# yinyunie/Pose2Room

Hardware: AMD Instinct MI355X
Metric: P2RNet train-step samples/sec (T=1024,J=53,bs=32) (higher is better)
Workload: dtype f32; 1 GPU; P2RNet full train step, bs=32/GPU, T=1024, J=53, seeds=512, proposals=128 (BASELINE configs[2]); input=P2RNet_dataloader over SyntheticPoseDataset, global_batch=32, frames=1024, parallelism=dp1

## Files before the change

include/p2r_hip.h:

```cpp
#ifndef P2R_HIP_H
#define P2R_HIP_H

#include <stdint.h>

#ifdef __cplusplus
extern "C" {
#endif

#define P2R_OK 0
#define P2R_EINVAL (-22)

int p2r_abi_version(void);
const char *p2r_build_arch(void);


int p2r_furthest_point_sampling(int b, int n, int m, const float *dataset,
                                float *temp, int *idxs, void *stream);

int p2r_gather_points(int b, int c, int n, int npoints, const float *points,
                      const int *idx, float *out, void *stream);

int p2r_gather_points_grad(int b, int c, int n, int npoints,
                           const float *grad_out, const int *idx,
                           float *grad_points, void *stream);
// ... 63 lines not shown

int p2r_stgcn_gcn_forward(int N, int T, int V, int K, const int *Lk_host,
                          const float *x, const float *W, const uint8_t *nbr,
                          const float *coef, const float *bias_cv, float *z,
                          float *stats_partial, void *stream);

int p2r_stgcn_gcn2_forward(int N, int T, int V, int K, int ltot, const float *x, const float *Wp,
                           const float *coef, const int *stream, int *stream_work,
                           const float *bias_cv, const float *addend, float *z, float *stats_partial,
                           int *n_partials, const float *bwd_u, const unsigned char *bwd_mask,
                           const float *bwd_fin, void *stream_h);

unsigned long long p2r_stgcn_gcn3_signature(int form);
int p2r_stgcn_gcn3_forward(int N, int T, int V, int K, int ltot, int form, const float *x, const float *Wp,
                           const float *coef, const float *bias_cv, const float *addend, float *z,
                           float *stats_partial, int *n_partials, const float *bwd_u,
                           const unsigned char *bwd_mask, const float *bwd_fin, void *stream_h);

int p2r_stgcn_gcn3_data_gradient_masked_addend(int N, int T, int V, int K, int ltot, const float *x,
                                               const float *Wp, const float *coef, const float *addend,
                                               const unsigned char *addend_mask, float *z, float *stats_partial,
                                               const float *bwd_u, const unsigned char *bwd_mask,
                                               const float *bwd_fin, void *stream_h);

int p2r_stgcn_gcn3_coef_grad(int N, int T, int V, int K, int ltot, const float *x, const float *dz,
                             const float *Wp, int n_blocks, float *dcoef_partial, void *stream);

int p2r_stgcn_gcn3_weight_grad(int N, int T, int V, int K, int ltot, const float *x, const float *dz,
                               const float *coef, int n_blocks, float *dw_partial, float *colsum_partial,
                               void *stream);

int p2r_stgcn_gcn_weight_grad(int N, int T, int V, int K, const int *Lk_host,
                              const float *x, const float *dz,
                              const uint8_t *nbr, const float *coef,
                              int n_blocks, float *dw_partial, float *colsum_partial,
                              int colsum_of_x, void *stream);

int p2r_stgcn_gcn_coef_grad(int N, int T, int V, int K, const int *Lk_host,
                            const float *x, const float *dz, const float *Wt,
                            const uint8_t *nbr, const float *coef, int n_blocks,
                            float *dcoef_partial, void *stream);


int p2r_bn_stats(int rows, int L, const float *x, float *partial, void *stream);

int p2r_bn_apply(int N, int C, int L, const float *x, const float *scale,
// ... 218 lines not shown
```

pose2room_amd/_lib.py:

```python
import ctypes
import os
import re

_HERE = os.path.dirname(os.path.abspath(__file__))
LIB_PATH = os.environ.get("P2R_LIB_PATH") or os.path.join(_HERE, "libp2r_hip.so")
HEADER_PATH = os.path.join(os.path.dirname(_HERE), "include", "p2r_hip.h")

ABI_VERSION = 3

_lib = None


class P2RLibraryError(RuntimeError):
    pass


def declared_symbols(header_path=HEADER_PATH):
    with open(header_path) as f:
        text = f.read()
    text = re.sub(r"/\*.*?\*/", "", text, flags=re.S)
    return sorted(set(re.findall(r"\b(p2r_[a-z0-9_]+)\s*\(", text)))


def lib():
    global _lib
    if _lib is None:
        if not os.path.exists(LIB_PATH):
            raise P2RLibraryError(
                f"{LIB_PATH} is missing: build it with `python -c 'import __graft_entry__ as g; g.build()'` "
                "(or `make -C pose2room_amd/csrc`). pose2room_amd has no CPU fallback.")
# ... 47 lines not shown
```

pose2room_amd/csrc/stgcn_gcn3.hip:

```cpp
#include "stgcn_tile.h"

#include "gcn3_sched.inc"

#ifdef P2R_CYCLE_TRACE
__device__ unsigned long long g3_trace[8 * 32];
extern "C" int p2r_debug_g3_trace(unsigned long long *dst) {
  return (int)hipMemcpyFromSymbol(dst, HIP_SYMBOL(g3_trace), sizeof(g3_trace));
}
#define G3_TRACE_TILE(tile) const bool trace_on = blockIdx.x == 7 && (tile) == 7 + 3 * (int)gridDim.x
#define G3_MARK(i) do { if (trace_on && lane == 0) g3_trace[wave * 32 + (i)] = __builtin_readcyclecounter(); } while (0)
#else
#define G3_TRACE_TILE(tile)
#define G3_MARK(i)
#endif
namespace {

constexpr int G3_F = TILE_F, G3_CP = TILE_CP, G3_NPH = TILE_NPH, G3_NW = TILE_NW, G3_SLOTS = TILE_SLOTS;
constexpr int G3_RS = TILE_RS, G3_BUF = TILE_BUF, G3_NV4 = TILE_NV4, G3_PW = TILE_PW;
static_assert(G3_V == TILE_V && G3_K == 11, "schedule generated for another skeleton");

struct G3Params {
  int T;
  int tiles_per_seq, total_tiles;
};

constexpr int g3_slot_joints[2][G3_NW][G3_SLOTS] = {G3_SLOT_JOINTS_0, G3_SLOT_JOINTS_1};
constexpr int g3_plane0[2][G3_NW] = {G3_PLANE0_0, G3_PLANE0_1};
constexpr int g3_first_slot(int form, int w) {
  for (int i = 0; i < G3_SLOTS; ++i)
    if (g3_slot_joints[form][w][i] >= 0) return i;
  return 0;
}
constexpr int g3_wave_joints(int form, int w) {
  int n = 0;
  for (int i = 0; i < G3_SLOTS; ++i) n += g3_slot_joints[form][w][i] >= 0;
  return n;
}
constexpr int G3_ST = 3;

template <int NE, int O0, int O1, int O2, int O3, int O4, int O5>
__device__ __forceinline__ void g3_gather(const char *xl, float (&xv)[6][4]) {
  constexpr int off[6] = {O0, O1, O2, O3, O4, O5};
#pragma unroll
  for (int j = 0; j < NE; ++j)
#pragma unroll
    for (int s = 0; s < 4; ++s) xv[j][s] = *reinterpret_cast<const float *>(xl + off[j] + s * 4 * G3_RS * 4);
}
// ... 48 lines not shown
  {                                                                              \
    float xv_[6][4], cf_[6];                                                     \
    g3_gather<ne, o0, o1, o2, o3, o4, o5>(xl, xv_);                              \
    g3_coefs<ne, c0, c1, c2, c3, c4, c5>(cl, cf_);                               \
    __builtin_amdgcn_sched_barrier(0);                                           \
    G3_MFMA(set, slot)                                                           \
    __builtin_amdgcn_sched_barrier(0);                                           \
    g3_combine<ne>(cf_, xv_, b_cur);                                             \
  }
#define G3_LAST(set, slot)             \
  {                                    \
    __builtin_amdgcn_sched_barrier(0); \
    G3_MFMA(set, slot)                 \
  }
#define G3_END(parity, pieces, plane0)                                                    \
  {                                                                                       \
    if (copy) { _Pragma("unroll") for (int i_ = pieces; i_ < G3_PW; ++i_) dma_piece(i_); } \
    if (parity) {                                                                         \
      _Pragma("unroll") for (int m_ = 0; m_ < 4; ++m_) _Pragma("unroll") for (int s_ = 0; s_ < 4; ++s_) \
          aS[0][m_][s_] = aS[1][m_][s_];                                                  \
    }                                                                                     \
  }

template <int FORM, bool BWD, int WAVE, bool MADD = false>
__device__ __forceinline__ void g3_wave_main(
    const G3Params &p, float *lds, const float *__restrict__ x, const float *__restrict__ Wp,
    const float *__restrict__ addend, float *__restrict__ z, bool want_stats, const float *__restrict__ bwd_u,
    const unsigned char *__restrict__ bwd_mask, const unsigned char *__restrict__ addend_mask = nullptr) {
  constexpr int V = G3_V, RS = G3_RS, BUF = G3_BUF, NW = G3_NW, SLOTS = G3_SLOTS;
  constexpr int wave = WAVE;
  float *rowstat = lds + 2 * BUF;
  float *bias_l = rowstat + NW * 64 * G3_ST;
  float *bstat = bias_l + 64 * V;
  float *coef_l = bstat + 128;

  const int tid = threadIdx.x;
  const int lane = tid & 63;
  const int g = lane >> 4, r = lane & 15;

  constexpr const int (&sj)[SLOTS] = g3_slot_joints[FORM][WAVE];

  const size_t row_stride = (size_t)p.T * V;
  const char *xl0 = reinterpret_cast<const char *>(lds + g * RS + r * V);
  unsigned cl_off = (unsigned)((coef_l - lds) * sizeof(float));
  asm volatile("" : "+v"(cl_off));
  const char *cl = reinterpret_cast<const char *>(lds) + cl_off;

  int doff[G3_PW];
#pragma unroll
  for (int i = 0; i < G3_PW; ++i) {
    const int pc = i * NW + wave;
    const int e = pc * 64 + lane;
    const int row = e / (RS / 4), c4 = e - row * (RS / 4);
    doff[i] = (pc < TILE_PIECES && e < G3_NV4) ? (int)(((size_t)row * row_stride + 4 * c4) * sizeof(float)) : -1;
  }

  f32x4 acc[SLOTS][4];
  float aS[2][4][4];
  float b_cur[4];
  auto load_a = [&](float (&a)[4][4], int k, int ph) { tile_load_a(a, Wp, k, ph, lane); };

  int tile = blockIdx.x;
  if (tile < p.total_tiles) {
    const int seq = tile / p.tiles_per_seq, t0 = (tile % p.tiles_per_seq) * G3_F;
    const float *xr = x + (size_t)seq * 64 * row_stride + (size_t)t0 * V;
#pragma unroll
    for (int i = 0; i < G3_PW; ++i)
      if (doff[i] >= 0) tile_dma16(xr, doff[i], lds + (i * NW + wave) * 256);
  }
  load_a(aS[0], g3_plane0[FORM][WAVE], 0);

  for (; tile < p.total_tiles; tile += gridDim.x) {
    const int seq = tile / p.tiles_per_seq, t0 = (tile % p.tiles_per_seq) * G3_F;
    const float *xg = x + (size_t)seq * 64 * row_stride + (size_t)t0 * V;
    float *zg = z + (size_t)seq * 64 * row_stride + (size_t)t0 * V;
    const float *ag = addend ? addend + (size_t)seq * 64 * row_stride + (size_t)t0 * V : nullptr;
    const float *ug = BWD ? bwd_u + (size_t)seq * 64 * row_stride + (size_t)t0 * V : nullptr;
    const unsigned char *mg = BWD ? bwd_mask + (size_t)seq * 64 * row_stride + (size_t)t0 * V : nullptr;
    const unsigned char *amg = MADD ? addend_mask + (size_t)seq * 64 * row_stride + (size_t)t0 * V : nullptr;
    const int ntile = tile + gridDim.x;
    const bool has_next = ntile < p.total_tiles;
    const int nseq = has_next ? ntile / p.tiles_per_seq : 0, nt0 = has_next ? (ntile % p.tiles_per_seq) * G3_F : 0;
    const float *nxg = x + (size_t)nseq * 64 * row_stride + (size_t)nt0 * V;
    G3_TRACE_TILE(tile);
    G3_MARK(0);

#pragma unroll
    for (int i = 0; i < SLOTS; ++i) {
      const float *bl = bias_l + 4 * g * V + (sj[i] >= 0 ? sj[i] : 0);
#pragma unroll
      for (int m = 0; m < 4; ++m)
#pragma unroll
        for (int q = 0; q < 4; ++q) acc[i][m][q] = bl[(16 * m + q) * V];
    }

#pragma unroll 1
    for (int ph = 0; ph < G3_NPH; ++ph) {
      G3_MARK(1 + 3 * ph);
      asm volatile("s_waitcnt vmcnt(0)" ::: "memory");
      G3_MARK(2 + 3 * ph);
      __syncthreads();
      G3_MARK(3 + 3 * ph);
      float *buf_nxt = lds + ((ph + 1) & 1) * BUF;
      const char *xl = xl0 + (ph & 1) * BUF * sizeof(float);
      const bool copy = ph + 1 < G3_NPH || has_next;
      const float *src = (ph + 1 < G3_NPH) ? xg + (size_t)(ph + 1) * G3_CP * row_stride : nxg;
      auto dma_piece = [&](int i) {
        if (doff[i] >= 0) tile_dma16(src, doff[i], buf_nxt + (i * NW + wave) * 256);
      };

      if constexpr (FORM == 0) {
        if constexpr (WAVE == 0) { G3_BODY_0_0 } else if constexpr (WAVE == 1) { G3_BODY_0_1 }
        else if constexpr (WAVE == 2) { G3_BODY_0_2 } else if constexpr (WAVE == 3) { G3_BODY_0_3 }
        else if constexpr (WAVE == 4) { G3_BODY_0_4 } else if constexpr (WAVE == 5) { G3_BODY_0_5 }
        else if constexpr (WAVE == 6) { G3_BODY_0_6 } else { G3_BODY_0_7 }
      } else {
        if constexpr (WAVE == 0) { G3_BODY_1_0 } else if constexpr (WAVE == 1) { G3_BODY_1_1 }
        else if constexpr (WAVE == 2) { G3_BODY_1_2 } else if constexpr (WAVE == 3) { G3_BODY_1_3 }
        else if constexpr (WAVE == 4) { G3_BODY_1_4 } else if constexpr (WAVE == 5) { G3_BODY_1_5 }
        else if constexpr (WAVE == 6) { G3_BODY_1_6 } else { G3_BODY_1_7 }
      }
    }

    G3_MARK(13);
// ... 119 lines not shown
#pragma unroll
          for (int it = 0; it < (G3_NV4 + NW * 64 - 1) / (NW * 64); ++it) {
            const int e = it * NW * 64 + tid;
            if (e < G3_NV4) {
              const int row = e / (RS / 4), c4 = e - row * (RS / 4);
              float4 v = srow[e];
              if (arow) {
                const float4 ad4 = arow[(size_t)row * (row_stride / 4) + c4];
                v.x += ad4.x; v.y += ad4.y; v.z += ad4.z; v.w += ad4.w;
              }
              zrow[(size_t)row * (row_stride / 4) + c4] = v;
            }
          }
        }
        asm volatile("s_waitcnt lgkmcnt(0)" ::: "memory");
        __builtin_amdgcn_s_barrier();
      }
    }
    G3_MARK(15);
  }

}

template <int FORM, bool BWD, bool MADD = false>
__global__ __launch_bounds__(G3_NW * 64, 2) void gcn3_kernel(
    G3Params p, int ltot, const float *__restrict__ x, const float *__restrict__ Wp, const float *__restrict__ coef,
    const float *__restrict__ bias_cv, const float *__restrict__ addend, float *__restrict__ z,
    float *__restrict__ stats_partial, const float *__restrict__ bwd_u, const unsigned char *__restrict__ bwd_mask,
    const float *__restrict__ bwd_fin, const unsigned char *__restrict__ addend_mask) {
  constexpr int V = G3_V, BUF = G3_BUF, NW = G3_NW;
  extern __shared__ float lds[];
  float *rowstat = lds + 2 * BUF;
  float *bias_l = rowstat + NW * 64 * G3_ST;
  float *bstat = bias_l + 64 * V;
  float *coef_l = bstat + 128;
  const int tid = threadIdx.x;
  for (int e = tid; e < NW * 64 * G3_ST; e += NW * 64) rowstat[e] = 0.f;
  for (int e = tid; e < 64 * V; e += NW * 64) bias_l[e] = bias_cv ? bias_cv[e] : 0.f;
  for (int e = tid; e < ltot * V; e += NW * 64) coef_l[e] = coef[e];
  if (tid < 64) {
    bstat[2 * tid] = BWD ? bwd_fin[tid] : 0.f;
    bstat[2 * tid + 1] = BWD ? bwd_fin[64 + tid] : 1.f;
  }
  __syncthreads();

  const bool want_stats = stats_partial != nullptr;
  switch (__builtin_amdgcn_readfirstlane(tid >> 6)) {
    case 0: g3_wave_main<FORM, BWD, 0, MADD>(p, lds, x, Wp, addend, z, want_stats, bwd_u, bwd_mask, addend_mask); break;
    case 1: g3_wave_main<FORM, BWD, 1, MADD>(p, lds, x, Wp, addend, z, want_stats, bwd_u, bwd_mask, addend_mask); break;
    case 2: g3_wave_main<FORM, BWD, 2, MADD>(p, lds, x, Wp, addend, z, want_stats, bwd_u, bwd_mask, addend_mask); break;
    case 3: g3_wave_main<FORM, BWD, 3, MADD>(p, lds, x, Wp, addend, z, want_stats, bwd_u, bwd_mask, addend_mask); break;
    case 4: g3_wave_main<FORM, BWD, 4, MADD>(p, lds, x, Wp, addend, z, want_stats, bwd_u, bwd_mask, addend_mask); break;
    case 5: g3_wave_main<FORM, BWD, 5, MADD>(p, lds, x, Wp, addend, z, want_stats, bwd_u, bwd_mask, addend_mask); break;
    case 6: g3_wave_main<FORM, BWD, 6, MADD>(p, lds, x, Wp, addend, z, want_stats, bwd_u, bwd_mask, addend_mask); break;
    default: g3_wave_main<FORM, BWD, 7, MADD>(p, lds, x, Wp, addend, z, want_stats, bwd_u, bwd_mask, addend_mask); break;
  }

  if (stats_partial) {
    __syncthreads();
    if constexpr (BWD) {
      tile_write_sums<G3_ST>(rowstat, stats_partial, tid);
    } else if (tid < 64) {
      const int ntiles = (p.total_tiles - (int)blockIdx.x + (int)gridDim.x - 1) / (int)gridDim.x;
      const float per_joint = (float)(ntiles * G3_F);
      float nw[NW], mw[NW], qw[NW];
      float msum = 0.f;
#pragma unroll
      for (int w = 0; w < NW; ++w) {
        const float *e = rowstat + (w * 64 + tid) * G3_ST;
        nw[w] = per_joint * (float)g3_wave_joints(FORM, w);
        const float d = e[0] / nw[w];
        mw[w] = e[2] + d;
        qw[w] = fmaxf(e[1] - e[0] * d, 0.f);
        msum = fmaf(nw[w], mw[w] - mw[0], msum);
      }
      const float n = per_joint * (float)V;
      const float mean = mw[0] + msum / n;
      float m2 = 0.f;
#pragma unroll
      for (int w = 0; w < NW; ++w) m2 += qw[w] + nw[w] * (mw[w] - mean) * (mw[w] - mean);
      float *o = stats_partial + (size_t)blockIdx.x * 192 + 3 * tid;
      o[0] = n; o[1] = mean; o[2] = m2;
    }
  }
}

template <int FORM, bool BWD, bool MADD = false>
int gcn3_launch(const G3Params &p, int ltot, int blocks, size_t lds, const float *x, const float *Wp, const float *coef,
                const float *bias_cv, const float *addend, float *z, float *stats_partial, const float *bwd_u,
                const unsigned char *bwd_mask, const float *bwd_fin, void *stream_h,
                const unsigned char *addend_mask = nullptr) {
  return p2r_launch_big_lds<gcn3_kernel<FORM, BWD, MADD>>(blocks, G3_NW * 64, lds, stream_h, p, ltot, x, Wp, coef, bias_cv,
                                                          addend, z, stats_partial, bwd_u, bwd_mask, bwd_fin, addend_mask);
}

}

extern "C" unsigned long long p2r_stgcn_gcn3_signature(int form) {
  return form == 0 ? G3_SIGNATURE_0 : (form == 1 ? G3_SIGNATURE_1 : 0ull);
}

static int gcn3_forward_impl(int N, int T, int V, int K, int ltot, int form, const float *x, const float *Wp,
                             const float *coef, const float *bias_cv, const float *addend, float *z,
                             float *stats_partial, int *n_partials, const float *bwd_u,
                             const unsigned char *bwd_mask, const float *bwd_fin, const unsigned char *addend_mask,
                             void *stream_h) {
// ... 33 lines not shown
                                       bwd_fin, stream_h);
  return gcn3_launch<1, false>(p, ltot, blocks, lds, x, Wp, coef, bias_cv, addend, z, stats_partial, nullptr, nullptr, nullptr,
                               stream_h);
}

extern "C" int p2r_stgcn_gcn3_forward(int N, int T, int V, int K, int ltot, int form, const float *x, const float *Wp,
                                      const float *coef, const float *bias_cv, const float *addend, float *z,
                                      float *stats_partial, int *n_partials, const float *bwd_u,
                                      const unsigned char *bwd_mask, const float *bwd_fin, void *stream_h) {
  return gcn3_forward_impl(N, T, V, K, ltot, form, x, Wp, coef, bias_cv, addend, z, stats_partial, n_partials, bwd_u, bwd_mask,
                           bwd_fin, nullptr, stream_h);
}

extern "C" int p2r_stgcn_gcn3_data_gradient_masked_addend(int N, int T, int V, int K, int ltot, const float *x,
                                                          const float *Wp, const float *coef, const float *addend,
                                                          const unsigned char *addend_mask, float *z,
                                                          float *stats_partial, const float *bwd_u,
                                                          const unsigned char *bwd_mask, const float *bwd_fin,
                                                          void *stream_h) {
  if (!addend_mask) return P2R_EINVAL;
  return gcn3_forward_impl(N, T, V, K, ltot, 1, x, Wp, coef, nullptr, addend, z, stats_partial, nullptr, bwd_u, bwd_mask,
                           bwd_fin, addend_mask, stream_h);
}
```

pose2room_amd/p2rnet/bn_op.py:

```python
import ctypes

import torch
from torch.autograd import Function

from .. import _lib
from . import handoff, math_mode


def _rows(x):
    N, C = x.shape[0], x.shape[1]
    L = x.numel() // max(N * C, 1)
    return N, C, L


def _stats_partial(x):
    N, C, L = _rows(x)
    part = torch.empty((N, C, 3), dtype=torch.float32, device=x.device)
    with torch.cuda.device(x.device):
        _lib.check(_lib.lib().p2r_bn_stats(N * C, L, _lib.ptr(x), _lib.ptr(part), _lib.current_stream(x.device)),
                   "bn_stats")
    return part


def _stats(x):
# ... 40 lines not shown
    mean = tot[:, 0] / M
    var = (tot[:, 1] / M - mean * mean).clamp_(min=0.0)
    return mean, var, float(M)


def _apply(x, scale, shift, res, relu, want_mask=False):
    N, C, L = _rows(x)
    y = torch.empty_like(x)
    mask = torch.empty(x.shape, dtype=torch.uint8, device=x.device) if (want_mask and relu) else None
    with torch.cuda.device(x.device):
        if relu and want_mask and math_mode.split16() and x.dim() == 4 and N > 0:
            word = math_mode.new_word(x.device)
            _lib.check(_lib.lib().p2r_bn_apply_amax(N, C, L, _lib.ptr(x), _lib.ptr(scale), _lib.ptr(shift), _lib.ptr(res),
                                                    _lib.ptr(y), _lib.ptr(mask), _lib.ptr(word),
                                                    _lib.current_stream(x.device)), "bn_apply_amax")
            math_mode.announce(y, word)
        else:
            _lib.check(_lib.lib().p2r_bn_apply(N, C, L, _lib.ptr(x), _lib.ptr(scale), _lib.ptr(shift), _lib.ptr(res),
                                               int(relu), _lib.ptr(y), _lib.ptr(mask), _lib.current_stream(x.device)),
                       "bn_apply")
    return (y, mask) if want_mask else y


GATE_HOOK = None

OVERLAP_APPLY = True
OVERLAP_REDUCE = True
SIDE_INLINE = False
_SIDE = {}


def _side_stream(dev):
    key = (dev.type, dev.index if dev.index is not None else torch.cuda.current_device())
    st = _SIDE.get(key)
    if st is None:
        st = _SIDE[key] = torch.cuda.Stream(device=dev, priority=-1)
    return st


class BNLink(object):
    __slots__ = ('u', 'mask', 'fin', 'versions', 'used')

    def __init__(self):
        self.u = self.mask = self.fin = self.versions = None
        self.used = 0

    def attach(self, u, mask, fin):
        self.u, self.mask, self.fin = u, mask, fin
        self.versions = (u._version, mask._version, fin._version)

    def intact(self):
        return (self.u is not None and self.versions is not None and
                self.versions == (self.u._version, self.mask._version, self.fin._version))


class _FusedBNAct(Function):

    @staticmethod
    def forward(ctx, x, weight, bias, res, fin, relu, link=None, lazy_res=False):
        x = x.contiguous()
        res_c = res.contiguous() if res is not None else None
        y, mask = _apply(x, fin[2], fin[3], res_c, relu, want_mask=True)
        ctx.save_for_backward(x, mask, fin)
        ctx.relu = relu
        ctx.split = math_mode.split16() and relu and x.dim() == 4
        ctx.has_res = res is not None
        ctx.lazy_res = bool(lazy_res) and relu and res is not None
        ctx.link = link if relu else None
        if ctx.link is not None:
            link.attach(x, mask, fin)
        return y

    @staticmethod
    def backward(ctx, dy):
        x, mask, fin = ctx.saved_tensors
        mean, invstd, kscale = fin[0], fin[1], fin[2]
        mode = 3 if ctx.relu else 0
        dy = dy.contiguous()
        N, C, L = _rows(x)
        dev = x.device
        lib = _lib.lib()
        link, part, ready = ctx.link, None, None
        sums = handoff.take(dy, 'bn_sums') if link is not None else None
        if sums is not None and sums[0] is link:
            _, part, ready = sums
# ... 29 lines not shown
                                                    _lib.ptr(invstd), _lib.ptr(kscale), _lib.ptr(tot_[2]), _lib.ptr(tot_[3]),
                                                    mode, None, None, _lib.ptr(dx_), _lib.ptr(dres_),
                                                    _lib.current_stream(dev)), "bn_bwd_apply")
            return tot_, dx_, dres_, word_

        if side_ok and SIDE_INLINE:
            tot, dx, dres, word = apply_pass()
        elif side_ok:
            main, side = torch.cuda.current_stream(dev), _side_stream(dev)
            side.wait_event(ready)
            with torch.cuda.stream(side):
                tot, dx, dres, word = apply_pass()
                done = torch.cuda.Event()
                done.record(side)
            main.wait_event(done)
            for t_ in (tot, dx, dres, word):
                if t_ is not None:
                    t_.record_stream(main)
        else:
            tot, dx, dres, word = apply_pass()
        if ctx.lazy_res:
            handoff.put(dy, 'res_mask', mask)
            dres = dy
        return dx, tot[1], tot[0], dres, None, None, None, None


class _EvalBNAct(Function):

    @staticmethod
    def forward(ctx, x, scale, shift, res, relu):
        x = x.contiguous()
        y = _apply(x, scale.contiguous(), shift.contiguous(), res.contiguous() if res is not None else None, relu)
        ctx.save_for_backward(x, y, scale)
        ctx.relu, ctx.has_res = relu, res is not None
        return y

    @staticmethod
    def backward(ctx, dy):
        x, y, scale = ctx.saved_tensors
        g = dy * (y > 0) if ctx.relu else dy
        dims = [d for d in range(dy.dim()) if d != 1]
        dscale = dshift = None
        if ctx.needs_input_grad[1]:
            dscale = (g.double() * x).sum(dims).float()
        if ctx.needs_input_grad[2]:
            dshift = g.double().sum(dims).float()
        dx = g * scale.view(1, -1, *([1] * (dy.dim() - 2))) if ctx.needs_input_grad[0] else None
        return dx, dscale, dshift, (g if ctx.has_res else None), None


def supported(x, bn):
    return x.is_cuda and x.dtype == torch.float32 and bn.affine and bn.track_running_stats and x.dim() >= 3


def fused_bn_act(x, bn, res=None, relu=True, stats=None, link=None, lazy_res=False):
    if bn.training:
        part = _stats_partial(x.contiguous()) if stats is None else stats
        fin = finalize(part, x.numel() // x.shape[1], bn)
        if GATE_HOOK is not None and relu:
            GATE_HOOK(bn, x, fin[2], fin[3], res)
        y = _FusedBNAct.apply(x, bn.weight, bn.bias, res, fin, relu, link, lazy_res)
        if link is not None and relu:
            y._p2r_bn_link = link
        return y
    invstd = torch.rsqrt(bn.running_var + bn.eps)
    scale = bn.weight * invstd
    shift = bn.bias - bn.running_mean * scale
    if GATE_HOOK is not None and relu:
        GATE_HOOK(bn, x, scale.detach(), shift.detach(), res)
    return _EvalBNAct.apply(x, scale, shift, res, relu)
```

pose2room_amd/p2rnet/gcn_op.py:

```python
import ctypes

import torch
from torch.autograd import Function

from .. import _lib
from . import bn_op, gcn_tables, handoff, math_mode

_N_BLOCKS = 256


class GraphTables:

    def __init__(self, A):
        self.K, self.V = int(A.shape[0]), int(A.shape[1])
        self.nbr_c, self.gidx_c, self.Lk_c = gcn_tables.build(A, transpose=False)
        self.nbr_r, self.gidx_r, self.Lk_r = gcn_tables.build(A, transpose=True)
        self.LkA_c = (ctypes.c_int * self.K)(*self.Lk_c)
        self.LkA_r = (ctypes.c_int * self.K)(*self.Lk_r)
        self.stream_c = self.stream_r = None
        if self.V == 53 and self.K < 15:
            try:
                sc = gcn_tables.build_stream(self.nbr_c, self.gidx_c, self.Lk_c)[0]
                sr = gcn_tables.build_stream(self.nbr_r, self.gidx_r, self.Lk_r)[0]
                self.stream_c, self.stream_r = torch.from_numpy(sc), torch.from_numpy(sr)
# ... 67 lines not shown
        _lib.check(_lib.lib().p2r_stgcn_gcn_forward(
            N, T, V, tables.K, LkA, _lib.ptr(x), _lib.ptr(W), _lib.ptr(nbr), _lib.ptr(coef),
            _lib.ptr(bias_cv), _lib.ptr(z), _lib.ptr(part), _lib.current_stream(x.device)), "stgcn_gcn_forward")
    return (z, part) if want_stats else z


def permute_planes(W3):
    K = W3.shape[0]
    return W3.reshape(K, 4, 16, 4, 4, 4).permute(0, 3, 1, 5, 2, 4).contiguous()


USE_GEN3 = True
SPLIT_WEIGHT_GRAD = True
SPLIT_COEF_GRAD = True


def _gen3_able(x, z, addend, tables, bwd=None):
    return (USE_GEN3 and tables.gen3 and x.shape[0] > 0 and x.shape[2] % 16 == 0 and x.data_ptr() % 16 == 0
            and z.data_ptr() % 16 == 0 and (addend is None or addend.data_ptr() % 16 == 0)
            and (bwd is None or (bwd[0].data_ptr() % 16 == 0 and bwd[1].data_ptr() % 4 == 0)))


def _gcn2_forward(x, Wp, coef, stream, bias_cv, tables, want_stats=False, addend=None, bwd=None, form=None,
                  addend_mask=None):
    N, C, T, V = x.shape
    z = torch.empty_like(x)
    lib = _lib.lib()
    part = None
    ltot = coef.shape[0]
    with torch.cuda.device(x.device):
        st = _lib.current_stream(x.device)
        gen3 = form is not None and _gen3_able(x, z, addend, tables, bwd)
        if addend_mask is not None and not (gen3 and form == 1 and addend_mask.data_ptr() % 4 == 0):
            addend = addend * (addend_mask != 0)
            addend_mask = None
        if want_stats:
            part = torch.empty((min(N * ((T + 15) // 16), 256), C, 3 if gen3 and bwd is None else 2),
                               dtype=torch.float32, device=x.device)
        if gen3 and addend_mask is not None:
            bu, bm, bf = (bwd[0], bwd[1], bwd[2].contiguous()) if bwd is not None else (None, None, None)
            _lib.check(lib.p2r_stgcn_gcn3_data_gradient_masked_addend(
                N, T, V, tables.K, ltot, _lib.ptr(x), _lib.ptr(Wp), _lib.ptr(coef), _lib.ptr(addend), _lib.ptr(addend_mask),
                _lib.ptr(z), _lib.ptr(part), _lib.ptr(bu), _lib.ptr(bm), _lib.ptr(bf), st),
                "stgcn_gcn3_data_gradient_masked_addend")
            return (z, part) if want_stats else z
        if gen3:
            bu, bm, bf = (bwd[0], bwd[1], bwd[2].contiguous()) if bwd is not None else (None, None, None)
            _lib.check(lib.p2r_stgcn_gcn3_forward(N, T, V, tables.K, ltot, int(form), _lib.ptr(x), _lib.ptr(Wp),
                                                  _lib.ptr(coef), _lib.ptr(bias_cv), _lib.ptr(addend), _lib.ptr(z),
                                                  _lib.ptr(part), None, _lib.ptr(bu), _lib.ptr(bm), _lib.ptr(bf), st),
                       "stgcn_gcn3_forward")
            return (z, part) if want_stats else z
        work = torch.empty_like(stream)
        bu, bm, bf = (bwd[0], bwd[1], bwd[2].contiguous()) if bwd is not None else (None, None, None)
        _lib.check(lib.p2r_stgcn_gcn2_forward(N, T, V, tables.K, ltot, _lib.ptr(x), _lib.ptr(Wp), _lib.ptr(coef),
                                              _lib.ptr(stream), _lib.ptr(work), _lib.ptr(bias_cv), _lib.ptr(addend),
                                              _lib.ptr(z), _lib.ptr(part), None, _lib.ptr(bu), _lib.ptr(bm),
                                              _lib.ptr(bf), st), "stgcn_gcn2_forward")
    return (z, part) if want_stats else z


# ... 76 lines not shown
    return (z, part) if want_stats else z


def _gcn3h_data_gradient(dz, sp, coef, tables, addend, addend_mask, dz_word):
    N, C, T, V = dz.shape
    dx = torch.empty_like(dz)
    with torch.cuda.device(dz.device):
        _lib.check(_lib.lib().p2r_stgcn_gcn3h_data_gradient(
            N, T, V, tables.K, coef.shape[0], _lib.ptr(dz), _lib.ptr(sp.wh), _lib.ptr(sp.winv), _lib.ptr(coef),
            _lib.ptr(addend), _lib.ptr(addend_mask), _lib.ptr(dx), _lib.ptr(dz_word), _lib.current_stream(dz.device)),
            "stgcn_gcn3h_data_gradient")
    return dx


class _GraphConv(Function):
    @staticmethod
    def forward(ctx, x, weight, coef_c, coef_r, bias_cv, tables, want_stats=False, with_residual=False,
                bn_link=None, wp_f=None, wp_b=None, lazy_res=False, split=None):
        dev = x.device
        t = tables.on(dev)
        x = x.contiguous()
        W = weight.contiguous()
        ctx.split = ctx.x_word = None
        if split is None and math_mode.split16() and _gen3h_able(x, tables):
            W3 = W.view(tables.K, 64, 64)
            split = (SplitPlanes(*split_planes(W3, tables.pairs_c)),
                     SplitPlanes(*split_planes(W3, tables.pairs_r, transposed=True)),
                     SplitPlanes(*split_planes_coef_grad(W3)))
        if split is not None and _gen3h_able(x, tables):
            ctx.split = split
            ctx.x_word = math_mode.range_word(x)
            out = _gcn3h_forward(x, split[0], coef_c.contiguous(), bias_cv.contiguous(), tables, want_stats, ctx.x_word)
        elif tables.gen2:
            out = _gcn2_forward(x, wp_f if wp_f is not None else permute_planes(W.view(tables.K, 64, 64)),
                                coef_c.contiguous(), t['stream_c'], bias_cv.contiguous(), tables, want_stats, form=0)
        else:
            out = _gcn_forward(x, W, t['nbr_c'], coef_c.contiguous(), tables.LkA_c, bias_cv.contiguous(), tables,
                               want_stats)
        ctx.save_for_backward(x, W, coef_c, coef_r)
        ctx.tables = tables
        ctx.bn_link = bn_link
        ctx.wp_b = wp_b
        ctx.wp_f = wp_f
        ctx.n_out = 2 if want_stats else 1
        ctx.lazy_res = bool(lazy_res) and with_residual
        if want_stats:
            ctx.mark_non_differentiable(out[1])
        if with_residual:
            out = (out if want_stats else (out,)) + (x.view_as(x),)
        return out

    @staticmethod
    def backward(ctx, dz, *rest):
        x, W, coef_c, coef_r = ctx.saved_tensors
        dres = rest[ctx.n_out - 1] if len(rest) >= ctx.n_out else None
        dres_mask = None
        if ctx.lazy_res and dres is not None:
            dres = dres.contiguous()
# ... 194 lines not shown
```

pose2room_amd/p2rnet/modules/stgcn.py:

```python
import torch
import torch.nn as nn

from ..registers import MODULES
from .stgcn_layers import Graph, st_gcn_block
from .sub_modules import SingleConv


def _point_mlp(cin, width, cout):
    return nn.Sequential(SingleConv(cin, width, kernel_size=1, order='cbr', padding=0, ndim=1),
                         SingleConv(width, width, kernel_size=1, order='cbr', padding=0, ndim=1),
                         SingleConv(width, cout, kernel_size=1, order='c', padding=0, ndim=1))


@MODULES.register_module
class STGCN(nn.Module):
    def __init__(self, cfg, optim_spec=None):
        super().__init__()
        self.optim_spec = optim_spec

        self.graph = Graph(layout='virtualroom', strategy='spatial', max_hop=5)
        self.register_buffer('A', torch.tensor(self.graph.A, dtype=torch.float32, requires_grad=False))

        self.n_seeds = cfg.config['data']['num_seeds']
        self.origin_joint_id = cfg.dataset_config.origin_joint_id
# ... 85 lines not shown
            torch.arange(-self.knn // 2, self.knn // 2, device=device).unsqueeze(0)
        win = win.clamp_(0, n_frames - 1)
        offs = hip[:, win] - hip.unsqueeze(2)
        pe = self._mlp(self.pos_embed, offs.reshape(n_batch, n_frames * self.knn, 3).transpose(1, 2).contiguous(), self.knn)
        from .. import seed_op
        pe = pe.view(n_batch, -1, n_frames, self.knn)
        fused = seed_op.short_rows_supported(pe)
        pe = seed_op.mean_last(pe) if fused else pe.mean(dim=3)
        rel = input_joints - input_joints[:, :, self.origin_joint_id:self.origin_joint_id + 1]
        sk = self._mlp(self.sk_feat, rel.reshape(n_batch, n_frames * n_joints, 3).transpose(1, 2).contiguous(), n_joints,
                       add_ct=pe)
        return sk.view(n_batch, -1, n_frames, n_joints)

    def forward(self, input_joints, end_points=None):
        end_points = {} if end_points is None else end_points
        n_batch, n_frames, n_joints, n_dim = input_joints.size()
        seed_inds = self._select_seeds(input_joints[:, :, self.origin_joint_id])

        x = self.embed(input_joints)
        blocks = self.st_gcn_networks
        tables = blocks[0].gcn.tables
        if tables is not None and tables.gen2 and all(b.chainable(x, self.A) for b in blocks):
            from ..gcn_op import prepare_chain
            for gcn, prep in zip(blocks, prepare_chain(blocks, self.A, self.edge_importance, tables, frames=x.shape[2])):
                x, _ = gcn(x, prep.Aeff, prepared=prep)
        else:
            for gcn, importance in zip(blocks, self.edge_importance):
                x, _ = gcn(x, self.A * importance)

        seed_skeleton = torch.gather(
            input_joints, 1, seed_inds[:, :, None, None].expand(n_batch, self.n_seeds, n_joints, n_dim))
        if self.n_seeds < n_frames:
            from .. import seed_op
            if seed_op.seed_rows_supported(x, seed_inds):
                rows = seed_op.seed_rows(x, seed_inds)
            else:
                rows = x.permute(0, 2, 1, 3)[torch.arange(n_batch, device=x.device)[:, None], seed_inds]
            seed_features = torch.nn.functional.linear(
                rows.reshape(n_batch, self.n_seeds, -1),
                self.conv_joint.weight.squeeze(-1), self.conv_joint.bias)
        else:
            x = x.transpose(2, 3).reshape(n_batch, -1, n_frames)
            seed_features = self.conv_joint(x).transpose(1, 2)
            seed_features = torch.gather(
                seed_features, 1, seed_inds.unsqueeze(-1).expand(n_batch, self.n_seeds, seed_features.size(-1)))
        end_points['seed_inds'] = seed_inds
        end_points['seed_skeleton'] = seed_skeleton[..., :3]
        end_points['seed_features'] = seed_features
# ... 2 lines not shown
```

pose2room_amd/p2rnet/modules/stgcn_layers.py:

```python
from collections import deque

import numpy as np
import torch
import torch.nn as nn

_VIRTUALROOM_BONES = [
    (0, 1), (1, 3), (3, 5), (5, 19), (0, 2), (2, 4), (4, 6), (6, 20), (0, 7), (7, 8), (8, 9),
    (9, 10), (10, 21), (10, 22), (8, 11), (11, 13), (13, 15), (15, 17), (8, 12), (12, 14),
    (14, 16), (16, 18), (17, 23), (23, 24), (24, 25), (17, 26), (26, 27), (27, 28), (17, 29),
    (29, 30), (30, 31), (17, 32), (32, 33), (33, 34), (17, 35), (35, 36), (36, 37), (18, 38),
    (38, 39), (39, 40), (18, 41), (41, 42), (42, 43), (18, 44), (44, 45), (45, 46), (18, 47),
    (47, 48), (48, 49), (18, 50), (50, 51), (51, 52)]

_LAYOUTS = {'virtualroom': dict(num_node=53, bones=_VIRTUALROOM_BONES, center=0)}


def hop_distance(num_node, edges, max_hop):
    nbr = [[] for _ in range(num_node)]
    for i, j in edges:
        if i != j:
            nbr[i].append(j)
            nbr[j].append(i)
    hop = np.full((num_node, num_node), np.inf)
    for s in range(num_node):
# ... 108 lines not shown
        if not residual:
            self.residual = _zero
        elif in_channels == out_channels and stride == 1:
            self.residual = _iden
        else:
            self.residual = nn.Sequential(
                nn.Conv2d(in_channels, out_channels, kernel_size=1, stride=(stride, 1)),
                nn.BatchNorm2d(out_channels))
        self.relu = nn.ReLU(inplace=True)

    fused_bn = True
    fused_tconv = True
    lazy_residual_grad = True
    chain_input = False

    def chainable(self, x, A):
        if not (self.fused_bn and x.is_cuda and self.tcn[4].p == 0):
            return False
        from .. import bn_op, gcn_op, tconv_op
        return (self.training and self.fused_tconv and self.gcn.tables is not None and self.gcn.fused
                and gcn_op.supported(x, self.gcn.conv.weight, A) and bn_op.supported(x, self.tcn[0])
                and tconv_op.supported(x, self.tcn[0], self.tcn[2]))

    def forward(self, x, A, prepared=None):
        res = self.residual(x)
        if self.fused_bn and x.is_cuda and self.tcn[4].p == 0:
            from .. import bn_op, gcn_op, tconv_op
            chain = self.chainable(x, A)
            assert chain or prepared is None
            lazy = False
            if chain:
                if self.residual is _iden and x.requires_grad:
                    in_link = getattr(x, '_p2r_bn_link', None) if self.chain_input else None
                    lazy = self.lazy_residual_grad and self.tcn[3].training
                    (z, zstats, res), A = self.gcn(x, A, want_stats=True, with_residual=True, bn_link=in_link,
                                                   prepared=prepared, lazy_res=lazy)
                else:
                    (z, zstats), A = self.gcn(x, A, want_stats=True, prepared=prepared)
                wp = (prepared.tcn_wp_f, prepared.tcn_wp_b) if prepared is not None and z.shape[3] == 53 else None
                u, ustats = tconv_op.bn_relu_tconv(z, self.tcn[0], self.tcn[2], stats=zstats, want_stats=True, wp=wp)
                res_t = res if torch.is_tensor(res) else None
                return bn_op.fused_bn_act(u, self.tcn[3], res_t, relu=True, stats=ustats, link=bn_op.BNLink(),
                                          lazy_res=lazy), A
            x, A = self.gcn(x, A)
            if bn_op.supported(x, self.tcn[0]):
                if self.fused_tconv and tconv_op.supported(x, self.tcn[0], self.tcn[2]):
                    u = tconv_op.bn_relu_tconv(x, self.tcn[0], self.tcn[2])
                else:
                    h = bn_op.fused_bn_act(x, self.tcn[0], None, relu=True)
                    u = self.tcn[2](h)
                res_t = res if torch.is_tensor(res) else None
                return bn_op.fused_bn_act(u, self.tcn[3], res_t, relu=True), A
        else:
            x, A = self.gcn(x, A)
        x = self.tcn(x) + res
        return self.relu(x), A
```

Baseline: 799.4 samples/s.

## Defer block-output BN apply and fuse it into next gcn3 forward load

Instead of running a standalone BatchNorm scale/shift + residual + ReLU pass at the end of each chained st_gcn block, the apply is recorded as a deferred handoff and executed inside the next block's gen3 graph-conv forward kernel. Each tile is transformed in LDS after loading, and the kernel also writes the materialized activation and the ReLU mask. This removes one kernel launch and one full read/write pass of the activation per intermediate block. In exchange it adds residual loads and extra stores inside the GEMM pipeline, which may lengthen the per-phase critical path. Consumers that cannot fuse fall back to a standalone apply.

```diff
diff --git a/include/p2r_hip.h b/include/p2r_hip.h
--- a/include/p2r_hip.h
+++ b/include/p2r_hip.h
@@ -109,6 +109,11 @@
                                                const unsigned char *addend_mask, float *z, float *stats_partial,
                                                const float *bwd_u, const unsigned char *bwd_mask,
                                                const float *bwd_fin, void *stream_h);
+
+int p2r_stgcn_gcn3_forward_xform(int N, int T, int V, int K, int ltot, const float *t, const float *scale,
+                                 const float *shift, const float *res, float *x_next, unsigned char *mask,
+                                 const float *Wp, const float *coef, const float *bias_cv, float *z,
+                                 float *stats_partial, int *n_partials, void *stream_h);
 
 int p2r_stgcn_gcn3_coef_grad(int N, int T, int V, int K, int ltot, const float *x, const float *dz,
                              const float *Wp, int n_blocks, float *dcoef_partial, void *stream);
diff --git a/pose2room_amd/_lib.py b/pose2room_amd/_lib.py
--- a/pose2room_amd/_lib.py
+++ b/pose2room_amd/_lib.py
@@ -6,6 +6,7 @@
 LIB_PATH = os.environ.get("P2R_LIB_PATH") or os.path.join(_HERE, "libp2r_hip.so")
 HEADER_PATH = os.path.join(os.path.dirname(_HERE), "include", "p2r_hip.h")
 
+P2R_EINVAL = -22
 ABI_VERSION = 3
 
 _lib = None
diff --git a/pose2room_amd/csrc/stgcn_gcn3.hip b/pose2room_amd/csrc/stgcn_gcn3.hip
--- a/pose2room_amd/csrc/stgcn_gcn3.hip
+++ b/pose2room_amd/csrc/stgcn_gcn3.hip
@@ -13,6 +13,9 @@
 #define G3_TRACE_TILE(tile)
 #define G3_MARK(i)
 #endif
+#ifndef G3X_RES_WARM
+#define G3X_RES_WARM 0
+#endif
 namespace {
 
 constexpr int G3_F = TILE_F, G3_CP = TILE_CP, G3_NPH = TILE_NPH, G3_NW = TILE_NW, G3_SLOTS = TILE_SLOTS;
@@ -23,6 +26,13 @@
   int T;
   int tiles_per_seq, total_tiles;
 };
+struct G3Xform {
+  const float *scale, *shift;
+  const float *res;
+  float *y;
+  unsigned char *mask;
+};
+typedef float g3_f4v __attribute__((ext_vector_type(4)));
 
 constexpr int g3_slot_joints[2][G3_NW][G3_SLOTS] = {G3_SLOT_JOINTS_0, G3_SLOT_JOINTS_1};
 constexpr int g3_plane0[2][G3_NW] = {G3_PLANE0_0, G3_PLANE0_1};
@@ -117,11 +127,11 @@
     }                                                                                     \
   }
 
-template <int FORM, bool BWD, int WAVE, bool MADD = false>
+template <int FORM, bool BWD, int WAVE, bool MADD = false, int XF = 0>
 __device__ __forceinline__ void g3_wave_main(
     const G3Params &p, float *lds, const float *__restrict__ x, const float *__restrict__ Wp,
     const float *__restrict__ addend, float *__restrict__ z, bool want_stats, const float *__restrict__ bwd_u,
-    const unsigned char *__restrict__ bwd_mask, const unsigned char *__restrict__ addend_mask = nullptr) {
+    const unsigned char *__restrict__ bwd_mask, const unsigned char *__restrict__ addend_mask, const G3Xform &xf) {
   constexpr int V = G3_V, RS = G3_RS, BUF = G3_BUF, NW = G3_NW, SLOTS = G3_SLOTS;
   constexpr int wave = WAVE;
   float *rowstat = lds + 2 * BUF;
@@ -155,6 +165,7 @@
   float b_cur[4];
   auto load_a = [&](float (&a)[4][4], int k, int ph) { tile_load_a(a, Wp, k, ph, lane); };
 
+  float xwarm = 0.f;
   int tile = blockIdx.x;
   if (tile < p.total_tiles) {
     const int seq = tile / p.tiles_per_seq, t0 = (tile % p.tiles_per_seq) * G3_F;
@@ -177,6 +188,8 @@
     const bool has_next = ntile < p.total_tiles;
     const int nseq = has_next ? ntile / p.tiles_per_seq : 0, nt0 = has_next ? (ntile % p.tiles_per_seq) * G3_F : 0;
     const float *nxg = x + (size_t)nseq * 64 * row_stride + (size_t)nt0 * V;
+    const size_t xf_tile = (size_t)seq * 64 * row_stride + (size_t)t0 * V;
+    const size_t xf_ntile = (size_t)nseq * 64 * row_stride + (size_t)nt0 * V;
     G3_TRACE_TILE(tile);
     G3_MARK(0);
 
@@ -192,9 +205,52 @@
 #pragma unroll 1
     for (int ph = 0; ph < G3_NPH; ++ph) {
       G3_MARK(1 + 3 * ph);
+      constexpr int XR4 = RS / 4, XIT = (XR4 + 31) / 32;
+      const int xcol = lane & 31, xrow = 2 * wave + (lane >> 5);
+      const size_t xf_off = xf_tile + (size_t)(G3_CP * ph + xrow) * row_stride + 4 * xcol;
+      g3_f4v xres[XF == 2 ? XIT : 1];
+      if constexpr (XF == 2) {
+        const g3_f4v *r4 = reinterpret_cast<const g3_f4v *>(xf.res + xf_off);
+#pragma unroll
+        for (int it = 0; it < XIT; ++it)
+          if (32 * it + 31 < XR4 || 32 * it + xcol < XR4) xres[it] = __builtin_nontemporal_load(r4 + 32 * it);
+      }
       asm volatile("s_waitcnt vmcnt(0)" ::: "memory");
+      if constexpr (XF == 2 && G3X_RES_WARM) asm volatile("" : "+v"(xwarm));
       G3_MARK(2 + 3 * ph);
       __syncthreads();
+      if constexpr (XF != 0) {
+        const int ch = G3_CP * ph + xrow;
+        const float sc = bstat[2 * ch], sh = bstat[2 * ch + 1];
+        float4 *rp = reinterpret_cast<float4 *>(lds + (ph & 1) * BUF + xrow * RS) + xcol;
+        g3_f4v *y4 = reinterpret_cast<g3_f4v *>(xf.y + xf_off);
+        uchar4 *m4 = reinterpret_cast<uchar4 *>(xf.mask + xf_off);
+#pragma unroll
+        for (int it = 0; it < XIT; ++it)
+          if (32 * it + 31 < XR4 || 32 * it + xcol < XR4) {
+            float4 v = rp[32 * it];
+            v.x = fmaf(v.x, sc, sh); v.y = fmaf(v.y, sc, sh); v.z = fmaf(v.z, sc, sh); v.w = fmaf(v.w, sc, sh);
+            if constexpr (XF == 2) {
+              v.x += xres[it].x; v.y += xres[it].y; v.z += xres[it].z; v.w += xres[it].w;
+            }
+            v.x = fmaxf(v.x, 0.f); v.y = fmaxf(v.y, 0.f); v.z = fmaxf(v.z, 0.f); v.w = fmaxf(v.w, 0.f);
+            rp[32 * it] = v;
+            __builtin_nontemporal_store(g3_f4v{v.x, v.y, v.z, v.w}, y4 + 32 * it);
+            m4[32 * it] = make_uchar4(v.x > 0.f, v.y > 0.f, v.z > 0.f, v.w > 0.f);
+          }
+        asm volatile("s_waitcnt lgkmcnt(0)" ::: "memory");
+        __builtin_amdgcn_s_barrier();
+        if constexpr (XF == 2 && G3X_RES_WARM) {
+          if (ph + 1 < G3_NPH || has_next) {
+            const float *wp = xf.res + (ph + 1 < G3_NPH ? xf_off + (size_t)G3_CP * row_stride
+                                                        : xf_ntile + (size_t)xrow * row_stride + 4 * xcol);
+#pragma unroll
+            for (int it = 0; it < XIT; ++it)
+              if (32 * it + 31 < XR4 || 32 * it + xcol < XR4)
+                asm volatile("global_load_dword %0, %1, off offset:%2" : "+v"(xwarm) : "v"(wp), "n"(512 * it) : "memory");
+          }
+        }
+      }
       G3_MARK(3 + 3 * ph);
       float *buf_nxt = lds + ((ph + 1) & 1) * BUF;
       const char *xl = xl0 + (ph & 1) * BUF * sizeof(float);
@@ -360,6 +416,31 @@
 
 }
 
+template <int FORM>
+__device__ __forceinline__ void g3_merge_moments(const G3Params &p, const float *rowstat, float *stats_partial, int tid) {
+  constexpr int V = G3_V, NW = G3_NW;
+  const int ntiles = (p.total_tiles - (int)blockIdx.x + (int)gridDim.x - 1) / (int)gridDim.x;
+  const float per_joint = (float)(ntiles * G3_F);
+  float nw[NW], mw[NW], qw[NW];
+  float msum = 0.f;
+#pragma unroll
+  for (int w = 0; w < NW; ++w) {
+    const float *e = rowstat + (w * 64 + tid) * G3_ST;
+    nw[w] = per_joint * (float)g3_wave_joints(FORM, w);
+    const float d = e[0] / nw[w];
+    mw[w] = e[2] + d;
+    qw[w] = fmaxf(e[1] - e[0] * d, 0.f);
+    msum = fmaf(nw[w], mw[w] - mw[0], msum);
+  }
+  const float n = per_joint * (float)V;
+  const float mean = mw[0] + msum / n;
+  float m2 = 0.f;
+#pragma unroll
+  for (int w = 0; w < NW; ++w) m2 += qw[w] + nw[w] * (mw[w] - mean) * (mw[w] - mean);
+  float *o = stats_partial + (size_t)blockIdx.x * 192 + 3 * tid;
+  o[0] = n; o[1] = mean; o[2] = m2;
+}
+
 template <int FORM, bool BWD, bool MADD = false>
 __global__ __launch_bounds__(G3_NW * 64, 2) void gcn3_kernel(
     G3Params p, int ltot, const float *__restrict__ x, const float *__restrict__ Wp, const float *__restrict__ coef,
@@ -383,15 +464,16 @@
   __syncthreads();
 
   const bool want_stats = stats_partial != nullptr;
+  const G3Xform no_xf{};
   switch (__builtin_amdgcn_readfirstlane(tid >> 6)) {
-    case 0: g3_wave_main<FORM, BWD, 0, MADD>(p, lds, x, Wp, addend, z, want_stats, bwd_u, bwd_mask, addend_mask); break;
-    case 1: g3_wave_main<FORM, BWD, 1, MADD>(p, lds, x, Wp, addend, z, want_stats, bwd_u, bwd_mask, addend_mask); break;
-    case 2: g3_wave_main<FORM, BWD, 2, MADD>(p, lds, x, Wp, addend, z, want_stats, bwd_u, bwd_mask, addend_mask); break;
-    case 3: g3_wave_main<FORM, BWD, 3, MADD>(p, lds, x, Wp, addend, z, want_stats, bwd_u, bwd_mask, addend_mask); break;
-    case 4: g3_wave_main<FORM, BWD, 4, MADD>(p, lds, x, Wp, addend, z, want_stats, bwd_u, bwd_mask, addend_mask); break;
-    case 5: g3_wave_main<FORM, BWD, 5, MADD>(p, lds, x, Wp, addend, z, want_stats, bwd_u, bwd_mask, addend_mask); break;
-    case 6: g3_wave_main<FORM, BWD, 6, MADD>(p, lds, x, Wp, addend, z, want_stats, bwd_u, bwd_mask, addend_mask); break;
-    default: g3_wave_main<FORM, BWD, 7, MADD>(p, lds, x, Wp, addend, z, want_stats, bwd_u, bwd_mask, addend_mask); break;
+    case 0: g3_wave_main<FORM, BWD, 0, MADD>(p, lds, x, Wp, addend, z, want_stats, bwd_u, bwd_mask, addend_mask, no_xf); break;
+    case 1: g3_wave_main<FORM, BWD, 1, MADD>(p, lds, x, Wp, addend, z, want_stats, bwd_u, bwd_mask, addend_mask, no_xf); break;
+    case 2: g3_wave_main<FORM, BWD, 2, MADD>(p, lds, x, Wp, addend, z, want_stats, bwd_u, bwd_mask, addend_mask, no_xf); break;
+    case 3: g3_wave_main<FORM, BWD, 3, MADD>(p, lds, x, Wp, addend, z, want_stats, bwd_u, bwd_mask, addend_mask, no_xf); break;
+    case 4: g3_wave_main<FORM, BWD, 4, MADD>(p, lds, x, Wp, addend, z, want_stats, bwd_u, bwd_mask, addend_mask, no_xf); break;
+    case 5: g3_wave_main<FORM, BWD, 5, MADD>(p, lds, x, Wp, addend, z, want_stats, bwd_u, bwd_mask, addend_mask, no_xf); break;
+    case 6: g3_wave_main<FORM, BWD, 6, MADD>(p, lds, x, Wp, addend, z, want_stats, bwd_u, bwd_mask, addend_mask, no_xf); break;
+    default: g3_wave_main<FORM, BWD, 7, MADD>(p, lds, x, Wp, addend, z, want_stats, bwd_u, bwd_mask, addend_mask, no_xf); break;
   }
 
   if (stats_partial) {
@@ -420,6 +502,45 @@
       float *o = stats_partial + (size_t)blockIdx.x * 192 + 3 * tid;
       o[0] = n; o[1] = mean; o[2] = m2;
     }
+  }
+}
+
+template <bool RES>
+__global__ __launch_bounds__(G3_NW * 64, 2) void gcn3x_kernel(
+    G3Params p, int ltot, const float *__restrict__ t, G3Xform xf, const float *__restrict__ Wp,
+    const float *__restrict__ coef, const float *__restrict__ bias_cv, float *__restrict__ z,
+    float *__restrict__ stats_partial) {
+  constexpr int V = G3_V, BUF = G3_BUF, NW = G3_NW, XF = RES ? 2 : 1;
+  extern __shared__ float lds[];
+  float *rowstat = lds + 2 * BUF;
+  float *bias_l = rowstat + NW * 64 * G3_ST;
+  float *bstat = bias_l + 64 * V;
+  float *coef_l = bstat + 128;
+  const int tid = threadIdx.x;
+  for (int e = tid; e < NW * 64 * G3_ST; e += NW * 64) rowstat[e] = 0.f;
+  for (int e = tid; e < 64 * V; e += NW * 64) bias_l[e] = bias_cv ? bias_cv[e] : 0.f;
+  for (int e = tid; e < ltot * V; e += NW * 64) coef_l[e] = coef[e];
+  if (tid < 64) {
+    bstat[2 * tid] = xf.scale[tid];
+    bstat[2 * tid + 1] = xf.shift[tid];
+  }
+  __syncthreads();
+
+  const bool want_stats = stats_partial != nullptr;
+  switch (__builtin_amdgcn_readfirstlane(tid >> 6)) {
+    case 0: g3_wave_main<0, false, 0, false, XF>(p, lds, t, Wp, nullptr, z, want_stats, nullptr, nullptr, nullptr, xf); break;
+    case 1: g3_wave_main<0, false, 1, false, XF>(p, lds, t, Wp, nullptr, z, want_stats, nullptr, nullptr, nullptr, xf); break;
+    case 2: g3_wave_main<0, false, 2, false, XF>(p, lds, t, Wp, nullptr, z, want_stats, nullptr, nullptr, nullptr, xf); break;
+    case 3: g3_wave_main<0, false, 3, false, XF>(p, lds, t, Wp, nullptr, z, want_stats, nullptr, nullptr, nullptr, xf); break;
+    case 4: g3_wave_main<0, false, 4, false, XF>(p, lds, t, Wp, nullptr, z, want_stats, nullptr, nullptr, nullptr, xf); break;
+    case 5: g3_wave_main<0, false, 5, false, XF>(p, lds, t, Wp, nullptr, z, want_stats, nullptr, nullptr, nullptr, xf); break;
+    case 6: g3_wave_main<0, false, 6, false, XF>(p, lds, t, Wp, nullptr, z, want_stats, nullptr, nullptr, nullptr, xf); break;
+    default: g3_wave_main<0, false, 7, false, XF>(p, lds, t, Wp, nullptr, z, want_stats, nullptr, nullptr, nullptr, xf); break;
+  }
+
+  if (stats_partial) {
+    __syncthreads();
+    if (tid < 64) g3_merge_moments<0>(p, rowstat, stats_partial, tid);
   }
 }
 
@@ -499,3 +620,35 @@
   return gcn3_forward_impl(N, T, V, K, ltot, 1, x, Wp, coef, nullptr, addend, z, stats_partial, nullptr, bwd_u, bwd_mask,
                            bwd_fin, addend_mask, stream_h);
 }
+
+extern "C" int p2r_stgcn_gcn3_forward_xform(int N, int T, int V, int K, int ltot, const float *t, const float *scale,
+                                            const float *shift, const float *res, float *x_next, unsigned char *mask,
+                                            const float *Wp, const float *coef, const float *bias_cv, float *z,
+                                            float *stats_partial, int *n_partials, void *stream_h) {
+  if (N < 0 || T <= 0 || V != G3_V || K != G3_K || ltot <= 0) return P2R_EINVAL;
+  if (T % G3_F != 0 || T > (1 << 20)) return P2R_EINVAL;
+  if (((uintptr_t)t % 16) != 0 || ((uintptr_t)z % 16) != 0 || ((uintptr_t)res % 16) != 0 ||
+      ((uintptr_t)x_next % 16) != 0 || ((uintptr_t)mask % 4) != 0)
+    return P2R_EINVAL;
+  if (n_partials) *n_partials = 0;
+  if (N == 0) return P2R_OK;
+  G3Params p;
+  p.T = T;
+  p.tiles_per_seq = T / G3_F;
+  const long long tiles = (long long)N * p.tiles_per_seq;
+  if (tiles > 0x7fffffffLL) return P2R_EINVAL;
+  p.total_tiles = (int)tiles;
+  const int blocks = (int)(tiles < 256 ? tiles : 256);
+  if (n_partials) *n_partials = blocks;
+  if (!z) return P2R_OK;
+  if (!t || !scale || !shift || !x_next || !mask || !Wp || !coef) return P2R_EINVAL;
+  const size_t lds = (size_t)2 * G3_BUF * sizeof(float) + (size_t)G3_NW * 64 * G3_ST * sizeof(float) +
+                     (size_t)64 * V * sizeof(float) + 128 * sizeof(float) + (size_t)ltot * V * sizeof(float);
+  if (lds > 160 * 1024) return P2R_EINVAL;
+  const G3Xform xf = {scale, shift, res, x_next, mask};
+  if (res)
+    return p2r_launch_big_lds<gcn3x_kernel<true>>(blocks, G3_NW * 64, lds, stream_h, p, ltot, t, xf, Wp, coef, bias_cv, z,
+                                                  stats_partial);
+  return p2r_launch_big_lds<gcn3x_kernel<false>>(blocks, G3_NW * 64, lds, stream_h, p, ltot, t, xf, Wp, coef, bias_cv, z,
+                                                 stats_partial);
+}
diff --git a/pose2room_amd/p2rnet/bn_op.py b/pose2room_amd/p2rnet/bn_op.py
--- a/pose2room_amd/p2rnet/bn_op.py
+++ b/pose2room_amd/p2rnet/bn_op.py
@@ -86,6 +86,49 @@
     return (y, mask) if want_mask else y
 
 
+DEFER_APPLY = True
+DEFER_COUNTS = {'fused': 0, 'standalone': 0}
+_warned_standalone = False
+
+
+def note_standalone(why):
+    global _warned_standalone
+    DEFER_COUNTS['standalone'] += 1
+    if not _warned_standalone:
+        _warned_standalone = True
+        import warnings
+        warnings.warn("bn_op: a deferred BatchNorm apply pass ran as a standalone launch (" + why + "); the step is "
+                      "correct but loses the fusion", RuntimeWarning, stacklevel=3)
+
+
+class DeferredApply(object):
+    __slots__ = ('t', 'scale', 'shift', 'res', 'mask')
+
+    def __init__(self, t, scale, shift, res, mask):
+        self.t, self.scale, self.shift, self.res, self.mask = t, scale, shift, res, mask
+
+    def run(self, y):
+        N, C, L = _rows(self.t)
+        with torch.cuda.device(y.device):
+            _lib.check(_lib.lib().p2r_bn_apply(N, C, L, _lib.ptr(self.t), _lib.ptr(self.scale), _lib.ptr(self.shift),
+                                               _lib.ptr(self.res), 1, _lib.ptr(y), _lib.ptr(self.mask),
+                                               _lib.current_stream(y.device)), "bn_apply")
+
+
+def materialize(y):
+    d = handoff.take(y, 'bn_deferred') if torch.is_tensor(y) else None
+    if d is not None:
+        note_standalone("its consumer is not a chainable st_gcn block")
+        d.run(y)
+    return y
+
+
+def defer_ok(x, tables):
+    from . import gcn_op
+    return (DEFER_APPLY and gcn_op.USE_GEN3 and tables is not None and tables.gen3 and not math_mode.split16()
+            and x.dim() == 4 and x.shape[0] > 0 and x.shape[2] % 16 == 0)
+
+
 GATE_HOOK = None
 
 OVERLAP_APPLY = True
@@ -121,10 +164,15 @@
 class _FusedBNAct(Function):
 
     @staticmethod
-    def forward(ctx, x, weight, bias, res, fin, relu, link=None, lazy_res=False):
+    def forward(ctx, x, weight, bias, res, fin, relu, link=None, lazy_res=False, defer=False):
         x = x.contiguous()
         res_c = res.contiguous() if res is not None else None
-        y, mask = _apply(x, fin[2], fin[3], res_c, relu, want_mask=True)
+        if defer and relu and x.dim() == 4 and x.shape[0] > 0 and not math_mode.split16():
+            y = torch.empty_like(x)
+            mask = torch.empty(x.shape, dtype=torch.uint8, device=x.device)
+            handoff.put(y, 'bn_deferred', DeferredApply(x, fin[2], fin[3], res_c, mask))
+        else:
+            y, mask = _apply(x, fin[2], fin[3], res_c, relu, want_mask=True)
         ctx.save_for_backward(x, mask, fin)
         ctx.relu = relu
         ctx.split = math_mode.split16() and relu and x.dim() == 4
@@ -200,7 +248,7 @@
         if ctx.lazy_res:
             handoff.put(dy, 'res_mask', mask)
             dres = dy
-        return dx, tot[1], tot[0], dres, None, None, None, None
+        return dx, tot[1], tot[0], dres, None, None, None, None, None
 
 
 class _EvalBNAct(Function):
@@ -231,13 +279,13 @@
     return x.is_cuda and x.dtype == torch.float32 and bn.affine and bn.track_running_stats and x.dim() >= 3
 
 
-def fused_bn_act(x, bn, res=None, relu=True, stats=None, link=None, lazy_res=False):
+def fused_bn_act(x, bn, res=None, relu=True, stats=None, link=None, lazy_res=False, defer=False):
     if bn.training:
         part = _stats_partial(x.contiguous()) if stats is None else stats
         fin = finalize(part, x.numel() // x.shape[1], bn)
         if GATE_HOOK is not None and relu:
             GATE_HOOK(bn, x, fin[2], fin[3], res)
-        y = _FusedBNAct.apply(x, bn.weight, bn.bias, res, fin, relu, link, lazy_res)
+        y = _FusedBNAct.apply(x, bn.weight, bn.bias, res, fin, relu, link, lazy_res, defer)
         if link is not None and relu:
             y._p2r_bn_link = link
         return y
diff --git a/pose2room_amd/p2rnet/gcn_op.py b/pose2room_amd/p2rnet/gcn_op.py
--- a/pose2room_amd/p2rnet/gcn_op.py
+++ b/pose2room_amd/p2rnet/gcn_op.py
@@ -113,7 +113,7 @@
 
 
 def _gcn2_forward(x, Wp, coef, stream, bias_cv, tables, want_stats=False, addend=None, bwd=None, form=None,
-                  addend_mask=None):
+                  addend_mask=None, deferred=None):
     N, C, T, V = x.shape
     z = torch.empty_like(x)
     lib = _lib.lib()
@@ -128,6 +128,20 @@
         if want_stats:
             part = torch.empty((min(N * ((T + 15) // 16), 256), C, 3 if gen3 and bwd is None else 2),
                                dtype=torch.float32, device=x.device)
+        if deferred is not None:
+            if gen3 and form == 0 and bwd is None and addend is None:
+                d = deferred
+                rc = lib.p2r_stgcn_gcn3_forward_xform(N, T, V, tables.K, ltot, _lib.ptr(d.t), _lib.ptr(d.scale),
+                                                      _lib.ptr(d.shift), _lib.ptr(d.res), _lib.ptr(x), _lib.ptr(d.mask),
+                                                      _lib.ptr(Wp), _lib.ptr(coef), _lib.ptr(bias_cv), _lib.ptr(z),
+                                                      _lib.ptr(part), None, st)
+                if rc == 0:
+                    bn_op.DEFER_COUNTS['fused'] += 1
+                    return (z, part) if want_stats else z
+                if rc != _lib.P2R_EINVAL:
+                    _lib.check(rc, "stgcn_gcn3_forward_xform")
+            bn_op.note_standalone("the graph conv that consumes it does not run on the fused third-generation forward")
+            deferred.run(x)
         if gen3 and addend_mask is not None:
             bu, bm, bf = (bwd[0], bwd[1], bwd[2].contiguous()) if bwd is not None else (None, None, None)
             _lib.check(lib.p2r_stgcn_gcn3_data_gradient_masked_addend(
@@ -250,18 +264,24 @@
         x = x.contiguous()
         W = weight.contiguous()
         ctx.split = ctx.x_word = None
+        deferred = handoff.take(x, 'bn_deferred')
         if split is None and math_mode.split16() and _gen3h_able(x, tables):
             W3 = W.view(tables.K, 64, 64)
             split = (SplitPlanes(*split_planes(W3, tables.pairs_c)),
                      SplitPlanes(*split_planes(W3, tables.pairs_r, transposed=True)),
                      SplitPlanes(*split_planes_coef_grad(W3)))
+        if deferred is not None and not (tables.gen2 and (split is None or not _gen3h_able(x, tables))):
+            bn_op.note_standalone("the graph conv that consumes it runs on the split16 or first-generation kernels")
+            deferred.run(x)
+            deferred = None
         if split is not None and _gen3h_able(x, tables):
             ctx.split = split
             ctx.x_word = math_mode.range_word(x)
             out = _gcn3h_forward(x, split[0], coef_c.contiguous(), bias_cv.contiguous(), tables, want_stats, ctx.x_word)
         elif tables.gen2:
             out = _gcn2_forward(x, wp_f if wp_f is not None else permute_planes(W.view(tables.K, 64, 64)),
-                                coef_c.contiguous(), t['stream_c'], bias_cv.contiguous(), tables, want_stats, form=0)
+                                coef_c.contiguous(), t['stream_c'], bias_cv.contiguous(), tables, want_stats, form=0,
+                                deferred=deferred)
         else:
             out = _gcn_forward(x, W, t['nbr_c'], coef_c.contiguous(), tables.LkA_c, bias_cv.contiguous(), tables,
                                want_stats)
diff --git a/pose2room_amd/p2rnet/modules/stgcn.py b/pose2room_amd/p2rnet/modules/stgcn.py
--- a/pose2room_amd/p2rnet/modules/stgcn.py
+++ b/pose2room_amd/p2rnet/modules/stgcn.py
@@ -131,8 +131,11 @@
         tables = blocks[0].gcn.tables
         if tables is not None and tables.gen2 and all(b.chainable(x, self.A) for b in blocks):
             from ..gcn_op import prepare_chain
-            for gcn, prep in zip(blocks, prepare_chain(blocks, self.A, self.edge_importance, tables, frames=x.shape[2])):
-                x, _ = gcn(x, prep.Aeff, prepared=prep)
+            from .. import bn_op
+            defer = bn_op.defer_ok(x, tables)
+            preps = prepare_chain(blocks, self.A, self.edge_importance, tables, frames=x.shape[2])
+            for i, (gcn, prep) in enumerate(zip(blocks, preps)):
+                x, _ = gcn(x, prep.Aeff, prepared=prep, defer_apply=defer and i + 1 < len(blocks))
         else:
             for gcn, importance in zip(blocks, self.edge_importance):
                 x, _ = gcn(x, self.A * importance)
diff --git a/pose2room_amd/p2rnet/modules/stgcn_layers.py b/pose2room_amd/p2rnet/modules/stgcn_layers.py
--- a/pose2room_amd/p2rnet/modules/stgcn_layers.py
+++ b/pose2room_amd/p2rnet/modules/stgcn_layers.py
@@ -154,11 +154,16 @@
                 and gcn_op.supported(x, self.gcn.conv.weight, A) and bn_op.supported(x, self.tcn[0])
                 and tconv_op.supported(x, self.tcn[0], self.tcn[2]))
 
-    def forward(self, x, A, prepared=None):
+    def forward(self, x, A, prepared=None, defer_apply=False):
+        chain = False
+        if x.is_cuda:
+            from .. import bn_op, gcn_op, tconv_op
+            chain = self.chainable(x, A)
+            if not chain:
+                bn_op.materialize(x)
+            assert self.residual is _iden or self.residual is _zero or bn_op.handoff.peek(x, 'bn_deferred') is None
         res = self.residual(x)
         if self.fused_bn and x.is_cuda and self.tcn[4].p == 0:
-            from .. import bn_op, gcn_op, tconv_op
-            chain = self.chainable(x, A)
             assert chain or prepared is None
             lazy = False
             if chain:
@@ -173,7 +178,7 @@
                 u, ustats = tconv_op.bn_relu_tconv(z, self.tcn[0], self.tcn[2], stats=zstats, want_stats=True, wp=wp)
                 res_t = res if torch.is_tensor(res) else None
                 return bn_op.fused_bn_act(u, self.tcn[3], res_t, relu=True, stats=ustats, link=bn_op.BNLink(),
-                                          lazy_res=lazy), A
+                                          lazy_res=lazy, defer=defer_apply), A
             x, A = self.gcn(x, A)
             if bn_op.supported(x, self.tcn[0]):
                 if self.fused_tconv and tconv_op.supported(x, self.tcn[0], self.tcn[2]):
```

New measurement: 816.5 samples/s (median of 6 runs). +2.1%, better.
